# max-andr/joint-cnn-mrf

Measured on AMD Instinct MI355X. Metric: images/sec (720x480, K=9 joints) part-detector+spatial-model fwd, higher is better.
Workload: dtype f32(fp16x2 spectra, fft); 1 GPU; configs[1]: batch=64/GPU synthetic 480x720x3, part detector + spatial model forward + argmax, fp32; batch_per_gpu=64, global_batch=64, micro_batch=64, use_sm=True, collective=all_gather coords int32 [B,2,9]

## Files before the change

joint-cnn-mrf_amd/csrc/conv_fft.hip:

```cpp
#include <cmath>
#include <cstdlib>
#include <map>
#include <mutex>
#include <utility>
#include <vector>

#include "conv_fft_common.h"

namespace jcm {
namespace cfft {

template <int KS, int NP>
__global__ __launch_bounds__(256) void weight_spectra_split_kernel(const float* __restrict__ w, uint4* __restrict__ Ws, int Cin, int Cout, int CoutP, int ntl, int NY, int NX,
                                                                   int round_bf16, float* __restrict__ wscale) {
  __shared__ cf twy[192][KS - 1], twx[KS];
  const int tid = threadIdx.x;
  const int kx = blockIdx.y;
#pragma unroll 1
  for (int k = tid; k < NY * (KS - 1) + KS; k += 256) {
    const bool isy = k < NY * (KS - 1);
    const int ky = k / (KS - 1), a = isy ? k % (KS - 1) + 1 : k - NY * (KS - 1);
    const int num = isy ? (ky * a) % NY : (kx * a) % NX, den = isy ? NY : NX;
    double sn, cs;
    sincospi(-2.0 * (double)num / (double)den, &sn, &cs);
// ... 276 lines not shown
  Sizes s;
  if (!sizes_of(a.H, a.W, ks, &s)) return 0;
  return (size_t)a.B * (s.NX / 2 + 1) * a.H * a.Cout * sizeof(cf);
}
bool conv_fft_win_gather_supported(int win, int Cin) { return fft_reg_on() && cfft_rows_fwd_win_reg_supported(win, Cin); }
bool conv_fft_win_scatter_supported(int win, int Cout) { return fft_reg_on() && win == 32 && Cout % 64 == 0; }
bool conv_fft_pool_fusable(const ConvArgs& a, int ks, int ks_next) {
  Sizes s, n;
  return sizes_of(a.H, a.W, ks, &s) && sizes_of((a.H + 1) / 2, (a.W + 1) / 2, ks_next, &n) && cfft_rows_inv_pool_fwd_supported(s.NX, n.NX, a.Cout);
}
size_t conv_fft_pool_handover_bytes(const ConvArgs& a, int ks_next) {
  Sizes n;
  if (!sizes_of((a.H + 1) / 2, (a.W + 1) / 2, ks_next, &n)) return 0;
  return (size_t)a.B * (n.NX / 2 + 1) * ((a.H + 1) / 2) * a.Cout * sizeof(cf);
}
bool conv_fft_tiles_supported(const ConvArgs& a, int ks, int ks_next) {
  Sizes s;
  return fft_reg_on() && fft_tiles_on() && ks == 5 && ks_next == 5 && !a.circ && !a.win_map && a.B >= 1 && conv_fft_pool_fusable(a, ks, ks_next) &&
         a.H % 4 == 0 && a.W % 4 == 0 && sizes_of(a.H / 2, a.W / 2, ks, &s) && cfft_tiles_supported(s.NY, s.NX, a);
}
bool conv_fft_merge_fusable(const ConvArgs& a, int ks, int ks_next, const FftMerge& m, bool h16) {
  Sizes s;
  if (!conv_fft_fusable(a, ks, ks_next) || !sizes_of(a.H, a.W, ks, &s)) return false;
  const bool reg = fft_reg_on() && cfft_rows_inv_merge_fwd_reg_supported(s.NX, a, m, (ks - 1) / 2);
  return h16 ? reg : (reg || cfft_rows_inv_merge_fwd_supported(s.NX, a, m));
}
static hipError_t conv_fft_tiles_f32(const ConvArgs& a0, int ks, int np, int in_layout, void* work, const FftLink& link, hipEvent_t g0, hipEvent_t g1, hipStream_t st,
                                     const Fp16Scale* scp) {
  const void* t_in = link.t_in; void* t_next = link.t_next; const FftMerge* merge = link.merge; void* xs = link.xs; const bool xs_ready = link.xs_ready; const FftNext* nx = &link.next;
  Sizes s;
  if (np != 4 || in_layout != 0 || t_in || merge || xs || xs_ready || !t_next || !nx || !nx->pool || nx->merge || !scp || !scp->tmax || !scp->winv || !scp->tmax_next ||
      !conv_fft_tiles_supported(a0, ks, nx->ks_next) || !sizes_of(a0.H / 2, a0.W / 2, ks, &s))
    return hipErrorInvalidValue;
  ConvArgs a = a0;
  a.CoutP = pad64(a.Cout);
  const ConvArgs at = tile_view(a, s);
  const Plan3 p = plan_of(at, s, np);
  Fp16Scale sc = *scp;
  sc.hf = (float)s.NY;
  sc.nb = at.B;
  char* wk = static_cast<char*>(work);
  cf* T = reinterpret_cast<cf*>(wk);
  void* Xs = wk + align256(p.t_bytes);
  cf* Yf = reinterpret_cast<cf*>(wk + align256(p.t_bytes) + align256(p.xs_bytes));
  int dev = 0;
  if (hipError_t e = hipGetDevice(&dev); e != hipSuccess) return e;
  const cf* twb = twiddle_table(dev);
  if (!twb) return hipErrorOutOfMemory;
  if (!cfft_rows_fwd_tile_reg(s.NY, s.NX, a, T, sc.tmax, st)) return hipErrorInvalidValue;
  if (hipError_t ce = cfft_cols_fwd(s.NY, at, np, T, Xs, twb + tw_offset(s.NY), p.NXH, p.MT, sc, st); ce != hipSuccess) return ce;
  if (hipError_t e = hipGetLastError(); e != hipSuccess) return e;
  if (g0 && hipEventRecord(g0, st) != hipSuccess) return hipErrorUnknown;
  if (hipError_t e = cgemm_split(Xs, a.wp, Yf, np, p.F, at.B, a.Cin, a.Cout, p.ldy, st, 0.f); e != hipSuccess) return e;
  if (g1 && hipEventRecord(g1, st) != hipSuccess) return hipErrorUnknown;
  ConvArgs ai = at;
  ai.H = a.H / 2;
  if (!cfft_cols_inv_reg(s.NY, ai, Yf, T, p.NXH, p.ldy, (ks - 1) / 2, st, nullptr, 0.f)) return hipErrorInvalidValue;
  if (!cfft_rows_inv_pool_tile_reg(s.NY, s.NX, a, T, static_cast<cf*>(t_next), 1.0f / (float)(s.NY * s.NX), sc, st)) return hipErrorInvalidValue;
  return hipGetLastError();
}
hipError_t conv_fft_f32(const ConvArgs& a0, int ks, int np, int in_layout, int out_layout, void* work, const FftLink& link, hipEvent_t g0, hipEvent_t g1, hipStream_t st,
                        const Fp16Scale* scp) {
  if (a0.tiles) return conv_fft_tiles_f32(a0, ks, np, in_layout, work, link, g0, g1, st, scp);
  const void* t_in = link.t_in; void* t_next = link.t_next; const FftMerge* merge = link.merge; void* xs = link.xs; const bool xs_ready = link.xs_ready; const FftNext* nx = &link.next;
  Sizes s;
  if (!conv_fft_supported(a0, ks) || !sizes_of(a0.H, a0.W, ks, &s, a0.circ) || (out_layout == 2 && a0.Cout % 8) || (np != 2 && np != 4 && np != 5) || (np == 5 && a0.Cin % 32)) return hipErrorInvalidValue;
  if (a0.circ && (t_in || t_next || merge || in_layout != 0 || out_layout != 0)) return hipErrorInvalidValue;
  if (nx && (nx->pool || nx->merge) && (!t_next || (nx->pool && nx->merge))) return hipErrorInvalidValue;
  Fp16Scale sc;
  if (np >= 4) {
    if (!scp || !scp->tmax || !scp->winv || (t_next && !scp->tmax_next)) return hipErrorInvalidValue;
    sc = *scp;
    sc.hf = (float)a0.H;
    sc.nb = a0.B;
  }
  const bool h16 = sc.t16 && ((t_next && nx && nx->merge && !t_in) || (t_in && !t_next));
  if ((t_in || t_next) && !h16 && (in_layout != 0 || out_layout != 0)) return hipErrorInvalidValue;
  if (t_next && a0.Cout % CB) return hipErrorInvalidValue;
  if (sc.t16 && (np != 5 || in_layout == 0 || out_layout == 0 || xs || ((t_in || t_next) && !h16))) return hipErrorInvalidValue;
  if (merge && in_layout == 2) return hipErrorInvalidValue;
  ConvArgs a = a0;
  a.CoutP = pad64(a.Cout);
  const int opad = (ks - 1) / 2 + (a0.circ ? 4 : 0);
  const Plan3 p = plan_of(a, s, np);
  char* wk = static_cast<char*>(work);
  cf* T = reinterpret_cast<cf*>(wk);
  void* Xs = xs ? xs : wk + align256(p.t_bytes);
  cf* Yf = reinterpret_cast<cf*>(wk + align256(p.t_bytes) + align256(p.xs_bytes));
  if (sc.t16) {
    sc.t16_fwd = reinterpret_cast<float*>(wk + align256(p.t_bytes) + align256(p.xs_bytes) + align256(p.yf_bytes));
    sc.t16_inv = reinterpret_cast<float*>(wk + align256(p.t_bytes) + align256(p.xs_bytes) + align256(p.yf_bytes) + align256(p.sc_fwd_bytes));
    sc.t16_cb = p.inv_cb;
    if (t_in) sc.t16_fwd = reinterpret_cast<float*>(const_cast<char*>(static_cast<const char*>(t_in)) + align256((size_t)a.B * p.NXH * a.H * a.Cin * 4));
  }
  if (xs_ready && !xs) return hipErrorInvalidValue;
  int dev = 0;
  if (hipError_t e = hipGetDevice(&dev); e != hipSuccess) return e;
  const cf* twb = twiddle_table(dev);
  if (!twb) return hipErrorOutOfMemory;
  const cf* twx = twb + tw_offset(s.NX);
  const cf* twy = twb + tw_offset(s.NY);
  const float norm = 1.0f / (float)(s.NY * s.NX);
  const cf* Tin = t_in ? static_cast<const cf*>(t_in) : T;
  const bool fft_reg = fft_reg_on();
  if (!xs_ready) {
    if (merge && !t_in) {
      if (!(fft_reg && cfft_rows_fwd_merge_reg(s.NX, a, *merge, in_layout, T, sc.tmax, st, sc.t16_fwd))) cfft_rows_fwd_merge(s.NX, a, *merge, in_layout, T, twx, sc.tmax, st, sc.t16_fwd);
    } else if (!t_in) {
      if (a.win_map) { if (!cfft_rows_fwd_win_reg(s.NX, a, T, sc.tmax, st)) return hipErrorInvalidValue; }
      else if (!(fft_reg && cfft_rows_fwd_reg(s.NX, a, in_layout, T, sc.tmax, st, sc.t16_fwd))) cfft_rows_fwd(s.NX, a, in_layout, T, twx, sc.tmax, st, sc.t16_fwd);
    }
    if (hipError_t ce = cfft_cols_fwd(s.NY, a, np, Tin, Xs, twy, p.NXH, p.MT, sc, st); ce != hipSuccess) return ce;
  }
  if (hipError_t e = hipGetLastError(); e != hipSuccess) return e;
  if (g0 && hipEventRecord(g0, st) != hipSuccess) return hipErrorUnknown;
  const float yshift = sc.t16 ? cgemm_split_y16_shift(a.Cin) : 0.f, yinv = yshift != 0.f ? 1.0f / yshift : 0.f;
  if (hipError_t e = cgemm_split(Xs, a.wp, Yf, np, p.F, a.B, a.Cin, a.Cout, p.ldy, st, yshift); e != hipSuccess) return e;
  if (g1 && hipEventRecord(g1, st) != hipSuccess) return hipErrorUnknown;
  ConvArgs ai = a;
  if (a0.circ) { ai.H = a0.H - 8; ai.W = a0.W - 8; }
  if (!(fft_reg && p.inv_cb == 64 && cfft_cols_inv_reg(s.NY, ai, Yf, T, p.NXH, p.ldy, opad, st, sc.t16_inv, yinv))) cfft_cols_inv(s.NY, ai, Yf, T, twy, p.NXH, p.ldy, opad, st, sc.t16_inv, yinv);
  if (t_next && nx && nx->pool) {
    Sizes sn;
    if (!sizes_of((a.H + 1) / 2, (a.W + 1) / 2, nx->ks_next, &sn) ||
        !cfft_rows_inv_pool_fwd(s.NX, sn.NX, a, T, static_cast<cf*>(t_next), twx, twb + tw_offset(sn.NX), opad, norm, sc, st))
      return hipErrorInvalidValue;
  } else if (t_next && nx && nx->merge) {
    if (sc.t16) {
      float* t16n = reinterpret_cast<float*>(static_cast<char*>(t_next) + align256((size_t)a.B * p.NXH * a.H * a.Cout * 4));
      if (!(fft_reg && cfft_rows_inv_merge_fwd_reg(s.NX, a, *nx->merge, T, static_cast<cf*>(t_next), opad, norm, sc, st, t16n))) return hipErrorInvalidValue;
    } else if (!(fft_reg && cfft_rows_inv_merge_fwd_reg(s.NX, a, *nx->merge, T, static_cast<cf*>(t_next), opad, norm, sc, st)) &&
               !cfft_rows_inv_merge_fwd(s.NX, a, *nx->merge, T, static_cast<cf*>(t_next), twx, opad, norm, sc, st)) {
      return hipErrorInvalidValue;
    }
  } else if (t_next) {
    if (!(fft_reg && cfft_rows_inv_fwd_reg(s.NX, a, T, static_cast<cf*>(t_next), opad, norm, sc, st))) cfft_rows_inv_fwd(s.NX, a, T, static_cast<cf*>(t_next), twx, opad, norm, sc, st);
  } else if (!((ai.rows_mfma & 1) && cfft_rows_inv_mfma(s.NX, ai, out_layout, T, opad, norm, sc, st)) && !(fft_reg && cfft_rows_inv_reg(s.NX, ai, out_layout, T, opad, norm, sc, st))) {
    if (ai.wout_TX > 0) return hipErrorInvalidValue;
    cfft_rows_inv(s.NX, ai, out_layout, T, twx, opad, norm, sc, st);
  }
  return hipGetLastError();
}

bool conv_fft_logits_rows_supported(const ConvArgs& a, int ks) {
  Sizes s;
  return fft_logits_rows_on() && ks == 9 && !a.circ && !a.tiles && !a.win_map && conv_fft_supported(a, ks) && sizes_of(a.H, a.W, ks, &s) && cfft_logits_rows_supported(s.NX, a);
}
size_t conv_fft_logits_weight_bytes(int H, int W, int Cin) {
  Sizes s;
  return sizes_of(H, W, 9, &s) ? cfft_logits_rows_operand_bytes(s.NX, Cin) : 0;
}
size_t conv_fft_logits_workspace_bytes(const ConvArgs& a) {
  Sizes s;
  return sizes_of(a.H, a.W, 9, &s) ? align256((size_t)a.B * a.H * (s.NX / 2 + 1) * CB * sizeof(cf)) : 0;
}
hipError_t conv_fft_logits_pack(const float* w_hwio, void* aop, int H, int W, int Cin, int Cout, hipStream_t st, float* wscale) {
  Sizes s;
  if (!sizes_of(H, W, 9, &s) || Cin % 16 || Cout > 16 || !wscale) return hipErrorInvalidValue;
  if (hipError_t e = hipMemsetAsync(wscale, 0, 2 * sizeof(float), st); e != hipSuccess) return e;
  const size_t pairs = (size_t)Cin * Cout;
  const dim3 bgrid((unsigned)((pairs + 255) / 256 > 1024 ? 1024 : (pairs + 255) / 256));
  hipLaunchKernelGGL(weight_bound_kernel<81>, bgrid, dim3(256), 0, st, w_hwio, pairs, 0, wscale);
  return cfft_logits_rows_pack(s.NX, w_hwio, aop, Cin, Cout, wscale, st);
}
hipError_t conv_fft_logits_f32(const ConvArgs& a0, void* work, const FftLink& link, hipEvent_t g0, hipEvent_t g1, hipStream_t st, const Fp16Scale* scp) {
  Sizes s;
  if (!conv_fft_logits_rows_supported(a0, 9) || !sizes_of(a0.H, a0.W, 9, &s) || !link.t_in || link.t_in_16 || link.t_next || link.merge || link.xs || link.xs_ready || link.win_scatter ||
      !scp || !scp->tmax || !scp->winv || scp->common)
    return hipErrorInvalidValue;
  ConvArgs a = a0;
  a.CoutP = pad64(a.Cout);
  Fp16Scale sc = *scp;
  sc.hf = 1.f;
  sc.nb = a.B;
  int dev = 0;
  if (hipError_t e = hipGetDevice(&dev); e != hipSuccess) return e;
  const cf* twb = twiddle_table(dev);
  if (!twb) return hipErrorOutOfMemory;
  cf* S = static_cast<cf*>(work);
  if (g0 && hipEventRecord(g0, st) != hipSuccess) return hipErrorUnknown;
  if (hipError_t e = cfft_logits_rows(s.NX, a, static_cast<const cf*>(link.t_in), a.wp, sc.tmax, S, st); e != hipSuccess) return e;
  if (g1 && hipEventRecord(g1, st) != hipSuccess) return hipErrorUnknown;
  cfft_rows_inv(s.NX, a, 0, S, twb + tw_offset(s.NX), 4, 1.0f / (float)s.NX, sc, st);
  return hipGetLastError();
}

size_t conv_fft_xs_bytes(const ConvArgs& a, int ks, int np) {
  Sizes s;
  if (!sizes_of(a.H, a.W, ks, &s, a.circ)) return 0;
  return align256(plan_of(a, s, np).xs_bytes);
}
hipError_t conv_fft_spectra(const ConvArgs& a0, int ks, int np, void* work, void* xs, hipStream_t st, float* tmax, int common) {
  Sizes s;
  if (!conv_fft_supported(a0, ks) || !sizes_of(a0.H, a0.W, ks, &s, a0.circ) || !xs || (np >= 4 && !tmax)) return hipErrorInvalidValue;
  Fp16Scale sc;
  if (np >= 4) { sc.tmax = tmax; sc.hf = (float)a0.H; sc.nb = a0.B; sc.common = common; }
  ConvArgs a = a0;
  a.CoutP = pad64(a.Cout);
  const Plan3 p = plan_of(a, s, np);
  int dev = 0;
  if (hipError_t e = hipGetDevice(&dev); e != hipSuccess) return e;
  const cf* twb = twiddle_table(dev);
  if (!twb) return hipErrorOutOfMemory;
  cf* T = static_cast<cf*>(work);
  if (a.win_map) { if (!cfft_rows_fwd_win_reg(s.NX, a, T, sc.tmax, st)) return hipErrorInvalidValue; }
  else cfft_rows_fwd(s.NX, a, 0, T, twb + tw_offset(s.NX), sc.tmax, st);
  if (hipError_t ce = cfft_cols_fwd(s.NY, a, np, T, xs, twb + tw_offset(s.NY), p.NXH, p.MT, sc, st); ce != hipSuccess) return ce;
  return hipGetLastError();
}
bool conv_fft_geometry(int H, int W, int ks, int B, int Cout, int np, int* NY, int* NX, int* MT, int circ) {
  Sizes s;
  if (!sizes_of(H, W, ks, &s, circ)) return false;
  *NY = s.NY; *NX = s.NX; *MT = cgemm_split_mtile(np, B, Cout);
  return true;
}

}
```

joint-cnn-mrf_amd/csrc/conv_fft_common.h:

```cpp
#pragma once
#include "fft_lds.h"
#include "kernels.h"

namespace jcm {
namespace cfft {
using namespace fftl;
constexpr int CB = 64, NT = 256;
constexpr int kParMax = 512;

template <int N> struct Plan;
template <> struct Plan<192> { static constexpr int R1 = 8, R2 = 8, R3 = 3; };
template <> struct Plan<128> { static constexpr int R1 = 8, R2 = 4, R3 = 4; };
template <> struct Plan<100> { static constexpr int R1 = 4, R2 = 5, R3 = 5; };
template <> struct Plan<96> { static constexpr int R1 = 8, R2 = 12, R3 = 1; };
template <> struct Plan<72> { static constexpr int R1 = 8, R2 = 3, R3 = 3; };
template <> struct Plan<64> { static constexpr int R1 = 8, R2 = 8, R3 = 1; };
template <> struct Plan<60> { static constexpr int R1 = 4, R2 = 15, R3 = 1; };
template <> struct Plan<50> { static constexpr int R1 = 5, R2 = 10, R3 = 1; };
template <> struct Plan<40> { static constexpr int R1 = 8, R2 = 5, R3 = 1; };
template <> struct Plan<36> { static constexpr int R1 = 4, R2 = 3, R3 = 3; };
template <> struct Plan<32> { static constexpr int R1 = 8, R2 = 4, R3 = 1; };
template <> struct Plan<28> { static constexpr int R1 = 4, R2 = 7, R3 = 1; };
template <> struct Plan<24> { static constexpr int R1 = 8, R2 = 3, R3 = 1; };
template <> struct Plan<20> { static constexpr int R1 = 4, R2 = 5, R3 = 1; };
// ... 105 lines not shown
  float4 o[K];
  float m = 0.f;
#pragma unroll
  for (int i = 0; i < K; ++i) {
    const int t = tid + i * NTH, k = t / CH, v = t % CH;
    o[i] = make_float4(0.f, 0.f, 0.f, 0.f);
    if (t < NXH * CH) {
      const cf zk = buf[pos<NX>(k) * CH + v], zn = buf[pos<NX>(k == 0 ? 0 : NX - k) * CH + v];
      o[i] = make_float4(0.5f * (zk.x + zn.x), 0.5f * (zk.y - zn.y), 0.5f * (zk.y + zn.y), -0.5f * (zk.x - zn.x));
      m = fmaxf(fmaxf(m, fmaxf(fabsf(o[i].x), fabsf(o[i].y))), fmaxf(fabsf(o[i].z), fabsf(o[i].w)));
    }
  }
  const float s = bfp_scale(block_max_all<NTH>(m, red2, tid));
#pragma unroll
  for (int i = 0; i < K; ++i) {
    const int t = tid + i * NTH, k = t / CH, v = t % CH;
    if (t < NXH * CH) dst[t_fwd_index(k, cblk, v, b, y, B, H, C)] = make_uint2(pack_h2(o[i].x * s, o[i].y * s), pack_h2(o[i].z * s, o[i].w * s));
  }
  if (tid == 0) tinv[((size_t)b * (C / CB) + cblk) * H + y] = 1.0f / s;
  return m;
}

constexpr int kFp16TargetExp = 15;
static_assert(kFp16TargetExp <= 15, "sqrt(2) * 2^kFp16TargetExp must stay below fp16's largest number 65504");
__device__ __forceinline__ int fp16_exp(float tmax, float hf) {
  const float bound = tmax * hf;
  int e = 0;
  if (bound > 0.f && bound < 3.0e38f) (void)frexpf(bound, &e);
  return e;
}
__device__ __forceinline__ int fp16_k(float tmax, float hf) { const int k = kFp16TargetExp - fp16_exp(tmax, hf); return k > 126 ? 126 : (k < -126 ? -126 : k); }
__device__ __forceinline__ float fp16_scale(float tmax, float hf) { return ldexpf(1.f, fp16_k(tmax, hf)); }
__device__ __forceinline__ float fp16_unscale(float tmax, float hf) { return ldexpf(1.f, -fp16_k(tmax, hf)); }
__device__ __forceinline__ float tmax_of(const float* __restrict__ tmax, int b, int nb, int common) {
  if (!common) return tmax[b];
  float m = 0.f;
  for (int i = 0; i < nb; ++i) m = fmaxf(m, tmax[i]);
  return m;
}
__device__ __forceinline__ void wave_max_stash(float m, float* red) {
#pragma unroll
  for (int o = 32; o > 0; o >>= 1) m = fmaxf(m, __shfl_xor(m, o));
  if ((threadIdx.x & 63) == 0) red[threadIdx.x >> 6] = m;
}
template <int NTH>
__device__ __forceinline__ void stash_to_word(const float* red, float* dst) {
  if (threadIdx.x == 0) {
    float m = red[0];
#pragma unroll
    for (int w = 1; w < NTH / 64; ++w) m = fmaxf(m, red[w]);
    if (m > 0.f) atomicMax(reinterpret_cast<unsigned*>(dst), __float_as_uint(m));
  }
}
template <int NTH>
__device__ __forceinline__ void block_max_to(float m, float* dst, float* red, int tid) {
#pragma unroll
  for (int o = 32; o > 0; o >>= 1) m = fmaxf(m, __shfl_xor(m, o));
  if ((tid & 63) == 0) red[tid >> 6] = m;
  __syncthreads();
  if (tid == 0) {
    for (int w = 1; w < NTH / 64; ++w) m = fmaxf(m, red[w]);
    if (m > 0.f) atomicMax(reinterpret_cast<unsigned*>(dst), __float_as_uint(m));
  }
}
template <int NX> constexpr int rows_threads() { return NX >= 128 ? 512 : NX >= 72 ? 384 : 256; }
template <int NY> constexpr int colblk() { return NY > 100 ? 32 : 64; }
template <int NY> constexpr int colimg() { return NY > 96 ? 4 : 8; }
template <int NY> constexpr int colfwd_threads() { return NY * colimg<NY>() * 16 >= 8192 ? 1024 : NY * colimg<NY>() * 16 >= 4096 ? 512 : 256; }
template <int NY> constexpr int colinv_threads() { return NY * colblk<NY>() >= 4096 ? 512 : 256; }
__device__ __forceinline__ void split8h(const float (&x)[8], float scale, uint4 (&out)[2]) {
  unsigned short h[2][8];
#pragma unroll
  for (int e = 0; e < 8; ++e) {
    float v = x[e] * scale;
#pragma unroll
    for (int p = 0; p < 2; ++p) {
      const _Float16 q = static_cast<_Float16>(v);
      h[p][e] = __builtin_bit_cast(unsigned short, q);
      v = v - static_cast<float>(q);
    }
  }
#pragma unroll
  for (int p = 0; p < 2; ++p)
    out[p] = make_uint4((unsigned)h[p][0] | ((unsigned)h[p][1] << 16), (unsigned)h[p][2] | ((unsigned)h[p][3] << 16), (unsigned)h[p][4] | ((unsigned)h[p][5] << 16),
                        (unsigned)h[p][6] | ((unsigned)h[p][7] << 16));
}
__device__ __forceinline__ uint4 round8h(const float (&x)[8], float scale) {
  unsigned short h[8];
#pragma unroll
  for (int e = 0; e < 8; ++e) h[e] = __builtin_bit_cast(unsigned short, static_cast<_Float16>(x[e] * scale));
  return make_uint4((unsigned)h[0] | ((unsigned)h[1] << 16), (unsigned)h[2] | ((unsigned)h[3] << 16), (unsigned)h[4] | ((unsigned)h[5] << 16), (unsigned)h[6] | ((unsigned)h[7] << 16));
}
template <int NP>
__device__ __forceinline__ void split8(const float (&x)[8], uint4 (&out)[NP]) {
  unsigned short h[NP][8];
#pragma unroll
  for (int e = 0; e < 8; ++e) {
    float v = x[e];
#pragma unroll
    for (int p = 0; p < NP; ++p) {
      const __bf16 q = static_cast<__bf16>(v);
      h[p][e] = __builtin_bit_cast(unsigned short, q);
      v = v - static_cast<float>(q);
    }
  }
#pragma unroll
  for (int p = 0; p < NP; ++p)
    out[p] = make_uint4((unsigned)h[p][0] | ((unsigned)h[p][1] << 16), (unsigned)h[p][2] | ((unsigned)h[p][3] << 16), (unsigned)h[p][4] | ((unsigned)h[p][5] << 16),
                        (unsigned)h[p][6] | ((unsigned)h[p][7] << 16));
}
#define CFFT_BY_SIZE(N, CALL)                    \
  switch (N) {                                   \
    case 20: CALL(20); break;                    \
    case 24: CALL(24); break;                    \
    case 28: CALL(28); break;                    \
    case 32: CALL(32); break;                    \
    case 36: CALL(36); break;                    \
    case 40: CALL(40); break;                    \
    case 50: CALL(50); break;                    \
    case 60: CALL(60); break;                    \
    case 64: CALL(64); break;                    \
    case 72: CALL(72); break;                    \
    case 96: CALL(96); break;                    \
    case 100: CALL(100); break;                  \
    case 128: CALL(128); break;                  \
    default: CALL(192); break;                   \
  }

int persistent_grid(const void* kernel, int ntiles, int threads, int dyn_lds = 0);

void cfft_rows_fwd(int NX, const ConvArgs& a, int layout, cf* T, const cf* tw, float* tmax, hipStream_t st, float* t16 = nullptr);
void cfft_rows_fwd_merge(int NX, const ConvArgs& a, const FftMerge& m, int in_layout, cf* T, const cf* tw, float* tmax, hipStream_t st, float* t16 = nullptr);
hipError_t cfft_cols_fwd(int NY, const ConvArgs& a, int np, const cf* T, void* Xs, const cf* tw, int NXH, int MT, const Fp16Scale& sc, hipStream_t st);
void cfft_cols_inv(int NY, const ConvArgs& a, const cf* Yf, cf* T, const cf* tw, int NXH, int ldy, int pad, hipStream_t st, float* t16 = nullptr, float y16_inv = 0.f);
void cfft_rows_inv(int NX, const ConvArgs& a, int layout, const cf* T, const cf* tw, int pad, float norm, const Fp16Scale& sc, hipStream_t st);
bool cfft_rows_inv_reg(int NX, const ConvArgs& a, int layout, const cf* T, int pad, float norm, const Fp16Scale& sc, hipStream_t st);
bool cfft_rows_inv_fwd_reg(int NX, const ConvArgs& a, const cf* T, cf* Tn, int pad, float norm, const Fp16Scale& sc, hipStream_t st);
bool cfft_rows_fwd_reg(int NX, const ConvArgs& a, int layout, cf* T, float* tmax, hipStream_t st, float* t16);
bool cfft_rows_fwd_win_reg(int NX, const ConvArgs& a, cf* T, float* tmax, hipStream_t st);
bool cfft_rows_fwd_win_reg_supported(int NX, int Cin);
bool cfft_tiles_supported(int NY, int NX, const ConvArgs& a);
bool cfft_rows_fwd_tile_reg(int NY, int NX, const ConvArgs& a, cf* T, float* tmax, hipStream_t st);
bool cfft_rows_inv_pool_tile_reg(int NY, int NX, const ConvArgs& a, const cf* T, cf* Tn, float norm, const Fp16Scale& sc, hipStream_t st);
bool cfft_rows_fwd_merge_reg(int NX, const ConvArgs& a, const FftMerge& m, int in_layout, cf* T, float* tmax, hipStream_t st, float* t16);
bool cfft_cols_inv_reg(int NY, const ConvArgs& a, const cf* Yf, cf* T, int NXH, int ldy, int pad, hipStream_t st, float* t16, float y16_inv = 0.f);
void cfft_rows_inv_fwd(int NX, const ConvArgs& a, const cf* T, cf* Tn, const cf* tw, int pad, float norm, const Fp16Scale& sc, hipStream_t st);
bool cfft_rows_inv_pool_fwd(int NXI, int NXO, const ConvArgs& a, const cf* T, cf* Tn, const cf* twi, const cf* two, int pad, float norm, const Fp16Scale& sc, hipStream_t st);
bool cfft_rows_inv_merge_fwd(int NX, const ConvArgs& a, const FftMerge& m, const cf* T, cf* Tn, const cf* tw, int pad, float norm, const Fp16Scale& sc, hipStream_t st);
bool cfft_rows_inv_merge_fwd_reg(int NX, const ConvArgs& a, const FftMerge& m, const cf* T, cf* Tn, int pad, float norm, const Fp16Scale& sc, hipStream_t st, float* t16n = nullptr);
bool cfft_rows_inv_merge_fwd_reg_supported(int NX, const ConvArgs& a, const FftMerge& m, int pad);
bool cfft_rows_inv_pool_fwd_supported(int NXI, int NXO, int Cout);
bool cfft_rows_inv_mfma(int NX, const ConvArgs& a, int layout, const cf* T, int pad, float norm, const Fp16Scale& sc, hipStream_t st);
bool cfft_rows_inv_merge_fwd_supported(int NX, const ConvArgs& a, const FftMerge& m);
bool cfft_logits_rows_supported(int NX, const ConvArgs& a);
size_t cfft_logits_rows_operand_bytes(int NX, int Cin);
hipError_t cfft_logits_rows_pack(int NX, const float* w_hwio, void* aop, int Cin, int Cout, float* wscale, hipStream_t st);
hipError_t cfft_logits_rows(int NX, const ConvArgs& a, const cf* T, const void* aop, const float* tmax, cf* S, hipStream_t st);
}
}
```

joint-cnn-mrf_amd/csrc/conv_fft_logits.hip:

```cpp
#include "conv_fft_common.h"

namespace jcm {
namespace cfft {

constexpr int kLrWaves = 8, kLrRows = 72, kLrUnits = 8;
constexpr int kLrLds = kLrWaves * kLrRows * kLrUnits * 16;
typedef _Float16 f16x8 __attribute__((ext_vector_type(8)));
typedef float f32x4 __attribute__((ext_vector_type(4)));

__device__ __forceinline__ int lr_slot(int r, int u) { return r * kLrUnits + (u ^ ((r >> 1) & 7)); }

__global__ __launch_bounds__(256) void logits_rows_operand_kernel(const float* __restrict__ w, uint4* __restrict__ Aop, int Cin, int Cout, int NX, float* __restrict__ wscale) {
  __shared__ cf twx[9];
  const int kx = blockIdx.y, KC = Cin >> 4;
  if (threadIdx.x < 9) {
    double sn, cs;
    sincospi(-2.0 * (double)((kx * (int)threadIdx.x) % NX) / (double)NX, &sn, &cs);
    twx[threadIdx.x] = cf{(float)cs, (float)sn};
  }
  __syncthreads();
  int ex = 0;
  const float bound = wscale[0];
  if (bound > 0.f && bound < 3.0e38f) (void)frexpf(bound, &ex);
  const float wmul = ldexpf(1.f, 14 - ex);
  if (blockIdx.x == 0 && blockIdx.y == 0 && threadIdx.x == 0) wscale[1] = ldexpf(1.f, ex - 14);
  const int e = blockIdx.x * 256 + threadIdx.x;
  if (e >= 9 * KC * 64) return;
  const int lane = e & 63, c = (e >> 6) % KC, dy = (e >> 6) / KC;
  const int j = lane & 15, g = lane >> 4, ch0 = c * 16 + (g & 1) * 8;
  cf a[8];
#pragma unroll
  for (int i = 0; i < 8; ++i) a[i] = cf{0.f, 0.f};
  if (j < Cout) {
#pragma unroll
    for (int b = 0; b < 9; ++b) {
      const float* tap = w + ((size_t)(dy * 9 + (8 - b)) * Cin + ch0) * Cout + j;
      const cf tw = twx[b];
#pragma unroll
      for (int i = 0; i < 8; ++i) a[i] = sfma(tap[(size_t)i * Cout], tw, a[i]);
    }
  }
  float vr[8], vi[8];
#pragma unroll
  for (int i = 0; i < 8; ++i) {
    vr[i] = g < 2 ? a[i].x : -a[i].y;
    vi[i] = g < 2 ? a[i].y : a[i].x;
  }
  uint4 u[2];
  uint4* dst = Aop + ((((size_t)kx * 9 + dy) * KC + c) * 4) * 64 + lane;
  split8h(vr, wmul, u);
  dst[0] = u[0]; dst[64] = u[1];
  split8h(vi, wmul, u);
  dst[128] = u[0]; dst[192] = u[1];
}

__global__ __launch_bounds__(512) __attribute__((amdgpu_waves_per_eu(4, 4))) void logits_rows_kernel(const float4* __restrict__ T, const uint4* __restrict__ Aop,
                                                                                                       const float* __restrict__ tmax, cf* __restrict__ S, int B, int H, int KC,
                                                                                                       int NXH, int per) {
  extern __shared__ __attribute__((aligned(16))) char lr_smem[];
  const int xcd = blockIdx.x & 7, slot = blockIdx.x >> 3, item = xcd * per + slot;
  if (slot >= per || item >= NXH * B) return;
  const int kx = item / B, b = item - kx * B;
  const int tid = threadIdx.x, wave = tid >> 6, lane = tid & 63;
  uint4* wl = reinterpret_cast<uint4*>(lr_smem) + wave * (kLrRows * kLrUnits);
  for (int i = lane; i < kLrRows * kLrUnits; i += 64) wl[i] = make_uint4(0u, 0u, 0u, 0u);
  const float scale = fp16_scale(tmax[b], 1.f);
  f32x4 sr[4], si[4];
#pragma unroll
  for (int m = 0; m < 4; ++m) { sr[m] = f32x4{0.f, 0.f, 0.f, 0.f}; si[m] = f32x4{0.f, 0.f, 0.f, 0.f}; }
  const int y0 = lane >> 1, y1 = 32 + (lane >> 1), hh = lane & 1;
  const bool in0 = y0 < H, in1 = y1 < H;
  float4 pre[2][4];
  auto fetch = [&](int c) __attribute__((always_inline)) {
    const float4* src = T + (((size_t)kx * KC + c) * B + b) * H * 8 + hh * 4;
#pragma unroll
    for (int q = 0; q < 4; ++q) {
      pre[0][q] = in0 ? src[(size_t)y0 * 8 + q] : make_float4(0.f, 0.f, 0.f, 0.f);
      pre[1][q] = in1 ? src[(size_t)y1 * 8 + q] : make_float4(0.f, 0.f, 0.f, 0.f);
    }
  };
  auto stash = [&](int i, int y) __attribute__((always_inline)) {
    float re[8], im[8];
#pragma unroll
    for (int q = 0; q < 4; ++q) { re[2 * q] = pre[i][q].x; im[2 * q] = pre[i][q].y; re[2 * q + 1] = pre[i][q].z; im[2 * q + 1] = pre[i][q].w; }
    uint4 ur[2], ui[2];
    split8h(re, scale, ur);
    split8h(im, scale, ui);
    const int r = y + 4;
    wl[lr_slot(r, hh)] = ur[0]; wl[lr_slot(r, 2 + hh)] = ui[0];
    wl[lr_slot(r, 4 + hh)] = ur[1]; wl[lr_slot(r, 6 + hh)] = ui[1];
  };
  const int g = lane >> 4, rl = lane & 15;
  if (wave < KC) fetch(wave);
  for (int c = wave; c < KC; c += kLrWaves) {
    if (in0) stash(0, y0);
    if (in1) stash(1, y1);
    if (c + kLrWaves < KC) fetch(c + kLrWaves);
    __builtin_amdgcn_fence(__ATOMIC_RELEASE, "wavefront");
    __builtin_amdgcn_wave_barrier();
    __builtin_amdgcn_fence(__ATOMIC_ACQUIRE, "wavefront");
    const uint4* bp = Aop + (((size_t)kx * 9 * KC + c) * 4) * 64 + lane;
#pragma unroll 3
    for (int dy = 0; dy < 9; ++dy) {
      const uint4* bq = bp + (size_t)dy * KC * 256;
      const f16x8 br0 = __builtin_bit_cast(f16x8, bq[0]), br1 = __builtin_bit_cast(f16x8, bq[64]);
      const f16x8 bi0 = __builtin_bit_cast(f16x8, bq[128]), bi1 = __builtin_bit_cast(f16x8, bq[192]);
#pragma unroll
      for (int m = 0; m < 4; ++m) {
        const int r = m * 16 + rl + dy;
        const f16x8 a0 = __builtin_bit_cast(f16x8, wl[lr_slot(r, g)]), a1 = __builtin_bit_cast(f16x8, wl[lr_slot(r, 4 + g)]);
        sr[m] = __builtin_amdgcn_mfma_f32_16x16x32_f16(a0, br1, sr[m], 0, 0, 0);
        si[m] = __builtin_amdgcn_mfma_f32_16x16x32_f16(a0, bi1, si[m], 0, 0, 0);
        sr[m] = __builtin_amdgcn_mfma_f32_16x16x32_f16(a1, br0, sr[m], 0, 0, 0);
        si[m] = __builtin_amdgcn_mfma_f32_16x16x32_f16(a1, bi0, si[m], 0, 0, 0);
        sr[m] = __builtin_amdgcn_mfma_f32_16x16x32_f16(a0, br0, sr[m], 0, 0, 0);
        si[m] = __builtin_amdgcn_mfma_f32_16x16x32_f16(a0, bi0, si[m], 0, 0, 0);
      }
    }
    __builtin_amdgcn_fence(__ATOMIC_RELEASE, "wavefront");
    __builtin_amdgcn_wave_barrier();
    __builtin_amdgcn_fence(__ATOMIC_ACQUIRE, "wavefront");
  }
  __syncthreads();
  float* red = reinterpret_cast<float*>(lr_smem);
#pragma unroll
  for (int m = 0; m < 4; ++m)
#pragma unroll
    for (int i = 0; i < 4; ++i) {
      red[(wave * 32 + m * 4 + i) * 64 + lane] = sr[m][i];
      red[(wave * 32 + 16 + m * 4 + i) * 64 + lane] = si[m][i];
    }
  __syncthreads();
  cf* Sb = S + ((size_t)b * H * NXH + kx) * 64;
#pragma unroll
  for (int q = 0; q < 2; ++q) {
    const int pi = tid + 512 * q, lo = pi & 63, mi = pi >> 6;
    float re = 0.f, im = 0.f;
#pragma unroll
    for (int wv = 0; wv < kLrWaves; ++wv) {
      re += red[(wv * 32 + mi) * 64 + lo];
      im += red[(wv * 32 + 16 + mi) * 64 + lo];
    }
    const int row = (mi >> 2) * 16 + (lo >> 4) * 4 + (mi & 3);
    if (row < H) Sb[(size_t)row * NXH * 64 + (lo & 15)] = cf{re, im};
  }
  for (int e = tid; e < H * 24; e += 512) {
    const int row = e / 24, q = e - row * 24;
    *reinterpret_cast<float4*>(Sb + (size_t)row * NXH * 64 + 16 + 2 * q) = make_float4(0.f, 0.f, 0.f, 0.f);
  }
}

bool cfft_logits_rows_supported(int NX, const ConvArgs& a) { return NX == 96 && a.H >= 1 && a.H <= 64 && a.Cin % 16 == 0 && a.Cout >= 1 && a.Cout <= 16 && a.B >= 1; }
size_t cfft_logits_rows_operand_bytes(int NX, int Cin) { return (size_t)(NX / 2 + 1) * 9 * (Cin / 16) * 4 * 64 * sizeof(uint4); }
hipError_t cfft_logits_rows_pack(int NX, const float* w_hwio, void* aop, int Cin, int Cout, float* wscale, hipStream_t st) {
  const dim3 grid((unsigned)((9 * (Cin / 16) * 64 + 255) / 256), (unsigned)(NX / 2 + 1));
  hipLaunchKernelGGL(logits_rows_operand_kernel, grid, dim3(256), 0, st, w_hwio, static_cast<uint4*>(aop), Cin, Cout, NX, wscale);
  return hipGetLastError();
}
hipError_t cfft_logits_rows(int NX, const ConvArgs& a, const cf* T, const void* aop, const float* tmax, cf* S, hipStream_t st) {
  if (!cfft_logits_rows_supported(NX, a)) return hipErrorInvalidValue;
  static LdsAttr attr;
  if (hipError_t e = attr.ensure(reinterpret_cast<const void*>(logits_rows_kernel), kLrLds); e != hipSuccess) return e;
  const int NXH = NX / 2 + 1, items = NXH * a.B, per = (items + 7) / 8;
  hipLaunchKernelGGL(logits_rows_kernel, dim3((unsigned)(per * 8)), dim3(512), kLrLds, st, reinterpret_cast<const float4*>(T), static_cast<const uint4*>(aop), tmax, S, a.B, a.H,
                     a.Cin / 16, NXH, per);
  return hipGetLastError();
}

}
}
```

Before: 7317 images/sec.

## Batch two images per logits-rows block, narrow spectra to 16 columns, add dedicated inverse

The logits channel-GEMM kernel now processes G=2 batch images per work group. Each weight operand fetched from global memory is reused across two images' MFMA chains, with grouped prefetch and sched barriers, at the cost of halved occupancy and doubled LDS. The spectrum buffer is narrowed from 64 to 16 complex columns per row, which removes the zero-padding stores. A new specialised inverse-row FFT kernel packs 4 rows per block into the transform's channel lanes to match the narrow layout. An environment variable can switch back to G=1.

```diff
diff --git a/joint-cnn-mrf_amd/csrc/conv_fft.hip b/joint-cnn-mrf_amd/csrc/conv_fft.hip
--- a/joint-cnn-mrf_amd/csrc/conv_fft.hip
+++ b/joint-cnn-mrf_amd/csrc/conv_fft.hip
@@ -452,7 +452,7 @@
 }
 size_t conv_fft_logits_workspace_bytes(const ConvArgs& a) {
   Sizes s;
-  return sizes_of(a.H, a.W, 9, &s) ? align256((size_t)a.B * a.H * (s.NX / 2 + 1) * CB * sizeof(cf)) : 0;
+  return sizes_of(a.H, a.W, 9, &s) ? align256((size_t)a.B * a.H * (s.NX / 2 + 1) * kLrCols * sizeof(cf)) : 0;
 }
 hipError_t conv_fft_logits_pack(const float* w_hwio, void* aop, int H, int W, int Cin, int Cout, hipStream_t st, float* wscale) {
   Sizes s;
@@ -468,8 +468,7 @@
   if (!conv_fft_logits_rows_supported(a0, 9) || !sizes_of(a0.H, a0.W, 9, &s) || !link.t_in || link.t_in_16 || link.t_next || link.merge || link.xs || link.xs_ready || link.win_scatter ||
       !scp || !scp->tmax || !scp->winv || scp->common)
     return hipErrorInvalidValue;
-  ConvArgs a = a0;
-  a.CoutP = pad64(a.Cout);
+  const ConvArgs& a = a0;
   Fp16Scale sc = *scp;
   sc.hf = 1.f;
   sc.nb = a.B;
@@ -481,8 +480,7 @@
   if (g0 && hipEventRecord(g0, st) != hipSuccess) return hipErrorUnknown;
   if (hipError_t e = cfft_logits_rows(s.NX, a, static_cast<const cf*>(link.t_in), a.wp, sc.tmax, S, st); e != hipSuccess) return e;
   if (g1 && hipEventRecord(g1, st) != hipSuccess) return hipErrorUnknown;
-  cfft_rows_inv(s.NX, a, 0, S, twb + tw_offset(s.NX), 4, 1.0f / (float)s.NX, sc, st);
-  return hipGetLastError();
+  return cfft_logits_rows_inv(s.NX, a, S, twb + tw_offset(s.NX), 4, 1.0f / (float)s.NX, sc, st);
 }
 
 size_t conv_fft_xs_bytes(const ConvArgs& a, int ks, int np) {
diff --git a/joint-cnn-mrf_amd/csrc/conv_fft_common.h b/joint-cnn-mrf_amd/csrc/conv_fft_common.h
--- a/joint-cnn-mrf_amd/csrc/conv_fft_common.h
+++ b/joint-cnn-mrf_amd/csrc/conv_fft_common.h
@@ -281,9 +281,11 @@
 bool cfft_rows_inv_pool_fwd_supported(int NXI, int NXO, int Cout);
 bool cfft_rows_inv_mfma(int NX, const ConvArgs& a, int layout, const cf* T, int pad, float norm, const Fp16Scale& sc, hipStream_t st);
 bool cfft_rows_inv_merge_fwd_supported(int NX, const ConvArgs& a, const FftMerge& m);
+constexpr int kLrCols = 16;
 bool cfft_logits_rows_supported(int NX, const ConvArgs& a);
 size_t cfft_logits_rows_operand_bytes(int NX, int Cin);
 hipError_t cfft_logits_rows_pack(int NX, const float* w_hwio, void* aop, int Cin, int Cout, float* wscale, hipStream_t st);
 hipError_t cfft_logits_rows(int NX, const ConvArgs& a, const cf* T, const void* aop, const float* tmax, cf* S, hipStream_t st);
-}
-}
+hipError_t cfft_logits_rows_inv(int NX, const ConvArgs& a, const cf* S, const cf* tw, int pad, float norm, const Fp16Scale& sc, hipStream_t st);
+}
+}
diff --git a/joint-cnn-mrf_amd/csrc/conv_fft_logits.hip b/joint-cnn-mrf_amd/csrc/conv_fft_logits.hip
--- a/joint-cnn-mrf_amd/csrc/conv_fft_logits.hip
+++ b/joint-cnn-mrf_amd/csrc/conv_fft_logits.hip
@@ -1,10 +1,15 @@
+#include <cstdlib>
+#include <type_traits>
+
 #include "conv_fft_common.h"
 
 namespace jcm {
 namespace cfft {
 
 constexpr int kLrWaves = 8, kLrRows = 72, kLrUnits = 8;
-constexpr int kLrLds = kLrWaves * kLrRows * kLrUnits * 16;
+constexpr int kLrSlice = kLrRows * kLrUnits;
+constexpr int kLrLds = kLrWaves * kLrSlice * 16;
+constexpr int kLrGroup = 2;
 typedef _Float16 f16x8 __attribute__((ext_vector_type(8)));
 typedef float f32x4 __attribute__((ext_vector_type(4)));
 
@@ -54,68 +59,108 @@
   dst[128] = u[0]; dst[192] = u[1];
 }
 
-__global__ __launch_bounds__(512) __attribute__((amdgpu_waves_per_eu(4, 4))) void logits_rows_kernel(const float4* __restrict__ T, const uint4* __restrict__ Aop,
-                                                                                                       const float* __restrict__ tmax, cf* __restrict__ S, int B, int H, int KC,
-                                                                                                       int NXH, int per) {
+template <int G>
+__global__ __launch_bounds__(512) __attribute__((amdgpu_waves_per_eu(4 / G, 4 / G))) void logits_rows_kernel(const float4* __restrict__ T, const uint4* __restrict__ Aop,
+                                                                                                               const float* __restrict__ tmax, cf* __restrict__ S, int B, int H,
+                                                                                                               int KC, int NXH, int per) {
   extern __shared__ __attribute__((aligned(16))) char lr_smem[];
+  const int NG = (B + G - 1) / G;
   const int xcd = blockIdx.x & 7, slot = blockIdx.x >> 3, item = xcd * per + slot;
-  if (slot >= per || item >= NXH * B) return;
-  const int kx = item / B, b = item - kx * B;
+  if (slot >= per || item >= NXH * NG) return;
+  const int kx = item / NG, b0 = (item - kx * NG) * G, ng = B - b0 < G ? B - b0 : G;
   const int tid = threadIdx.x, wave = tid >> 6, lane = tid & 63;
-  uint4* wl = reinterpret_cast<uint4*>(lr_smem) + wave * (kLrRows * kLrUnits);
-  for (int i = lane; i < kLrRows * kLrUnits; i += 64) wl[i] = make_uint4(0u, 0u, 0u, 0u);
-  const float scale = fp16_scale(tmax[b], 1.f);
-  f32x4 sr[4], si[4];
-#pragma unroll
-  for (int m = 0; m < 4; ++m) { sr[m] = f32x4{0.f, 0.f, 0.f, 0.f}; si[m] = f32x4{0.f, 0.f, 0.f, 0.f}; }
+  uint4* wl = reinterpret_cast<uint4*>(lr_smem) + wave * (G * kLrSlice);
+  for (int i = lane; i < G * kLrSlice; i += 64) wl[i] = make_uint4(0u, 0u, 0u, 0u);
+  float scale[G];
+  f32x4 sr[G][4], si[G][4];
+#pragma unroll
+  for (int gi = 0; gi < G; ++gi) {
+    scale[gi] = gi < ng ? fp16_scale(tmax[b0 + gi], 1.f) : 1.f;
+#pragma unroll
+    for (int m = 0; m < 4; ++m) { sr[gi][m] = f32x4{0.f, 0.f, 0.f, 0.f}; si[gi][m] = f32x4{0.f, 0.f, 0.f, 0.f}; }
+  }
   const int y0 = lane >> 1, y1 = 32 + (lane >> 1), hh = lane & 1;
   const bool in0 = y0 < H, in1 = y1 < H;
-  float4 pre[2][4];
+  float4 pre[G][2][4];
+  const int yl0 = in0 ? y0 : H - 1, yl1 = in1 ? y1 : H - 1;
   auto fetch = [&](int c) __attribute__((always_inline)) {
-    const float4* src = T + (((size_t)kx * KC + c) * B + b) * H * 8 + hh * 4;
-#pragma unroll
-    for (int q = 0; q < 4; ++q) {
-      pre[0][q] = in0 ? src[(size_t)y0 * 8 + q] : make_float4(0.f, 0.f, 0.f, 0.f);
-      pre[1][q] = in1 ? src[(size_t)y1 * 8 + q] : make_float4(0.f, 0.f, 0.f, 0.f);
+#pragma unroll
+    for (int gi = 0; gi < G; ++gi) {
+      const float4* src = T + (((size_t)kx * KC + c) * B + (gi < ng ? b0 + gi : B - 1)) * H * 8 + hh * 4;
+#pragma unroll
+      for (int q = 0; q < 4; ++q) {
+        pre[gi][0][q] = src[(size_t)yl0 * 8 + q];
+        pre[gi][1][q] = src[(size_t)yl1 * 8 + q];
+      }
     }
   };
-  auto stash = [&](int i, int y) __attribute__((always_inline)) {
+  auto stash = [&](int gi, int i, int y) __attribute__((always_inline)) {
     float re[8], im[8];
 #pragma unroll
-    for (int q = 0; q < 4; ++q) { re[2 * q] = pre[i][q].x; im[2 * q] = pre[i][q].y; re[2 * q + 1] = pre[i][q].z; im[2 * q + 1] = pre[i][q].w; }
+    for (int q = 0; q < 4; ++q) { re[2 * q] = pre[gi][i][q].x; im[2 * q] = pre[gi][i][q].y; re[2 * q + 1] = pre[gi][i][q].z; im[2 * q + 1] = pre[gi][i][q].w; }
     uint4 ur[2], ui[2];
-    split8h(re, scale, ur);
-    split8h(im, scale, ui);
+    split8h(re, scale[gi], ur);
+    split8h(im, scale[gi], ui);
     const int r = y + 4;
-    wl[lr_slot(r, hh)] = ur[0]; wl[lr_slot(r, 2 + hh)] = ui[0];
-    wl[lr_slot(r, 4 + hh)] = ur[1]; wl[lr_slot(r, 6 + hh)] = ui[1];
+    uint4* wg = wl + gi * kLrSlice;
+    wg[lr_slot(r, hh)] = ur[0]; wg[lr_slot(r, 2 + hh)] = ui[0];
+    wg[lr_slot(r, 4 + hh)] = ur[1]; wg[lr_slot(r, 6 + hh)] = ui[1];
   };
   const int g = lane >> 4, rl = lane & 15;
   if (wave < KC) fetch(wave);
   for (int c = wave; c < KC; c += kLrWaves) {
-    if (in0) stash(0, y0);
-    if (in1) stash(1, y1);
-    if (c + kLrWaves < KC) fetch(c + kLrWaves);
+#pragma unroll
+    for (int gi = 0; gi < G; ++gi) {
+      if (gi < ng) {
+        if (in0) stash(gi, 0, y0);
+        if (in1) stash(gi, 1, y1);
+      }
+    }
     __builtin_amdgcn_fence(__ATOMIC_RELEASE, "wavefront");
     __builtin_amdgcn_wave_barrier();
     __builtin_amdgcn_fence(__ATOMIC_ACQUIRE, "wavefront");
     const uint4* bp = Aop + (((size_t)kx * 9 * KC + c) * 4) * 64 + lane;
+    const bool more = c + kLrWaves < KC;
+    auto group = [&](int d3, auto dg, bool pf) __attribute__((always_inline)) {
+      constexpr int DG = decltype(dg)::value;
+      if constexpr (DG > 1) __builtin_amdgcn_sched_barrier(0);
+      uint4 bf[DG][4];
+#pragma unroll
+      for (int d = 0; d < DG; ++d)
+#pragma unroll
+        for (int f = 0; f < 4; ++f) bf[d][f] = bp[(size_t)(d3 + d) * KC * 256 + f * 64];
+      if (pf) fetch(c + kLrWaves);
+      if constexpr (DG > 1) __builtin_amdgcn_sched_barrier(0);
+#pragma unroll
+      for (int d = 0; d < DG; ++d) {
+        const int dy = d3 + d;
+        const f16x8 br0 = __builtin_bit_cast(f16x8, bf[d][0]), br1 = __builtin_bit_cast(f16x8, bf[d][1]);
+        const f16x8 bi0 = __builtin_bit_cast(f16x8, bf[d][2]), bi1 = __builtin_bit_cast(f16x8, bf[d][3]);
+#pragma unroll
+        for (int m = 0; m < 4; ++m) {
+          const int r = m * 16 + rl + dy;
+#pragma unroll
+          for (int gi = 0; gi < G; ++gi) {
+            const uint4* wg = wl + gi * kLrSlice;
+            const f16x8 a0 = __builtin_bit_cast(f16x8, wg[lr_slot(r, g)]), a1 = __builtin_bit_cast(f16x8, wg[lr_slot(r, 4 + g)]);
+            sr[gi][m] = __builtin_amdgcn_mfma_f32_16x16x32_f16(a0, br1, sr[gi][m], 0, 0, 0);
+            si[gi][m] = __builtin_amdgcn_mfma_f32_16x16x32_f16(a0, bi1, si[gi][m], 0, 0, 0);
+            sr[gi][m] = __builtin_amdgcn_mfma_f32_16x16x32_f16(a1, br0, sr[gi][m], 0, 0, 0);
+            si[gi][m] = __builtin_amdgcn_mfma_f32_16x16x32_f16(a1, bi0, si[gi][m], 0, 0, 0);
+            sr[gi][m] = __builtin_amdgcn_mfma_f32_16x16x32_f16(a0, br0, sr[gi][m], 0, 0, 0);
+            si[gi][m] = __builtin_amdgcn_mfma_f32_16x16x32_f16(a0, bi0, si[gi][m], 0, 0, 0);
+          }
+        }
+      }
+    };
+    using std::integral_constant;
+    if constexpr (G == 1) {
+      if (more) fetch(c + kLrWaves);
 #pragma unroll 3
-    for (int dy = 0; dy < 9; ++dy) {
-      const uint4* bq = bp + (size_t)dy * KC * 256;
-      const f16x8 br0 = __builtin_bit_cast(f16x8, bq[0]), br1 = __builtin_bit_cast(f16x8, bq[64]);
-      const f16x8 bi0 = __builtin_bit_cast(f16x8, bq[128]), bi1 = __builtin_bit_cast(f16x8, bq[192]);
-#pragma unroll
-      for (int m = 0; m < 4; ++m) {
-        const int r = m * 16 + rl + dy;
-        const f16x8 a0 = __builtin_bit_cast(f16x8, wl[lr_slot(r, g)]), a1 = __builtin_bit_cast(f16x8, wl[lr_slot(r, 4 + g)]);
-        sr[m] = __builtin_amdgcn_mfma_f32_16x16x32_f16(a0, br1, sr[m], 0, 0, 0);
-        si[m] = __builtin_amdgcn_mfma_f32_16x16x32_f16(a0, bi1, si[m], 0, 0, 0);
-        sr[m] = __builtin_amdgcn_mfma_f32_16x16x32_f16(a1, br0, sr[m], 0, 0, 0);
-        si[m] = __builtin_amdgcn_mfma_f32_16x16x32_f16(a1, bi0, si[m], 0, 0, 0);
-        sr[m] = __builtin_amdgcn_mfma_f32_16x16x32_f16(a0, br0, sr[m], 0, 0, 0);
-        si[m] = __builtin_amdgcn_mfma_f32_16x16x32_f16(a0, bi0, si[m], 0, 0, 0);
-      }
+      for (int dy = 0; dy < 9; ++dy) group(dy, integral_constant<int, 1>{}, false);
+    } else {
+#pragma unroll 1
+      for (int d3 = 0; d3 < 9; d3 += 3) group(d3, integral_constant<int, 3>{}, d3 == 6 && more);
     }
     __builtin_amdgcn_fence(__ATOMIC_RELEASE, "wavefront");
     __builtin_amdgcn_wave_barrier();
@@ -124,30 +169,81 @@
   __syncthreads();
   float* red = reinterpret_cast<float*>(lr_smem);
 #pragma unroll
-  for (int m = 0; m < 4; ++m)
-#pragma unroll
-    for (int i = 0; i < 4; ++i) {
-      red[(wave * 32 + m * 4 + i) * 64 + lane] = sr[m][i];
-      red[(wave * 32 + 16 + m * 4 + i) * 64 + lane] = si[m][i];
-    }
-  __syncthreads();
-  cf* Sb = S + ((size_t)b * H * NXH + kx) * 64;
-#pragma unroll
-  for (int q = 0; q < 2; ++q) {
-    const int pi = tid + 512 * q, lo = pi & 63, mi = pi >> 6;
-    float re = 0.f, im = 0.f;
-#pragma unroll
-    for (int wv = 0; wv < kLrWaves; ++wv) {
-      re += red[(wv * 32 + mi) * 64 + lo];
-      im += red[(wv * 32 + 16 + mi) * 64 + lo];
-    }
-    const int row = (mi >> 2) * 16 + (lo >> 4) * 4 + (mi & 3);
-    if (row < H) Sb[(size_t)row * NXH * 64 + (lo & 15)] = cf{re, im};
-  }
-  for (int e = tid; e < H * 24; e += 512) {
-    const int row = e / 24, q = e - row * 24;
-    *reinterpret_cast<float4*>(Sb + (size_t)row * NXH * 64 + 16 + 2 * q) = make_float4(0.f, 0.f, 0.f, 0.f);
-  }
+  for (int gi = 0; gi < G; ++gi)
+#pragma unroll
+    for (int m = 0; m < 4; ++m)
+#pragma unroll
+      for (int i = 0; i < 4; ++i) {
+        red[((gi * kLrWaves + wave) * 32 + m * 4 + i) * 64 + lane] = sr[gi][m][i];
+        red[((gi * kLrWaves + wave) * 32 + 16 + m * 4 + i) * 64 + lane] = si[gi][m][i];
+      }
+  __syncthreads();
+#pragma unroll
+  for (int gi = 0; gi < G; ++gi) {
+    if (gi >= ng) break;
+    cf* Sb = S + ((size_t)(b0 + gi) * H * NXH + kx) * kLrCols;
+    const float* rg = red + gi * (kLrWaves * 32 * 64);
+#pragma unroll
+    for (int q = 0; q < 2; ++q) {
+      const int pi = tid + 512 * q, lo = pi & 63, mi = pi >> 6;
+      float re = 0.f, im = 0.f;
+#pragma unroll
+      for (int wv = 0; wv < kLrWaves; ++wv) {
+        re += rg[(wv * 32 + mi) * 64 + lo];
+        im += rg[(wv * 32 + 16 + mi) * 64 + lo];
+      }
+      const int row = (mi >> 2) * 16 + (lo >> 4) * 4 + (mi & 3);
+      if (row < H) Sb[(size_t)row * NXH * kLrCols + (lo & 15)] = cf{re, im};
+    }
+  }
+}
+
+constexpr int kLiRows = 4;
+__global__ __launch_bounds__(rows_threads<96>()) void logits_rows_inv_kernel(const cf* __restrict__ S, float* __restrict__ out, const cf* __restrict__ twg, const float* __restrict__ bias,
+                                                                             const float* __restrict__ scale, const float* __restrict__ shift, int relu_bn, int BH, int H, int W, int Cout,
+                                                                             int pad, float norm0, Fp16Scale sc) {
+  constexpr int NX = 96, CH = CB / 2, NXH = NX / 2 + 1, NTR = rows_threads<NX>(), K = (NXH * CH + NTR - 1) / NTR, CP = kLrCols / 2;
+  static_assert(CH == kLiRows * CP, "the rows of a work group fill the transform's channel lanes");
+  __shared__ cf buf[NX * CH];
+  __shared__ cf tw[NX];
+  const int tid = threadIdx.x, by0 = blockIdx.x * kLiRows;
+  twiddles<NX, NTR>(tw, twg, tid);
+  const float4* src = reinterpret_cast<const float4*>(S);
+#pragma unroll
+  for (int i = 0; i < K; ++i) {
+    const int t = tid + i * NTR, k = t / CH, v = t % CH, by = by0 + v / CP;
+    if (t < NXH * CH) {
+      float4 q = by < BH ? src[((size_t)by * NXH + k) * CP + v % CP] : make_float4(0.f, 0.f, 0.f, 0.f);
+      const bool edge = k == 0 || k == NX / 2;
+      if (edge) { q.y = 0.f; q.w = 0.f; }
+      buf[k * CH + v] = cf{q.x - q.w, q.y + q.z};
+      if (!edge) buf[(NX - k) * CH + v] = cf{q.x + q.w, q.z - q.y};
+    }
+  }
+  __syncthreads();
+  fft<NX, 1, CH, NTR>(buf, tw, tid);
+  const int v = tid % CH, by = by0 + v / CP, c = 2 * (v % CP);
+  if (by < BH && c < Cout) {
+    const float ncommon = norm0 * sc.winv[0];
+    const float norm = ncommon * fp16_unscale(sc.tmax[by / H], sc.hf);
+    const bool two = c + 1 < Cout, pairs = (Cout & 1) == 0;
+    const float b0v = bias[c], b1v = two ? bias[c + 1] : 0.f;
+    float s0 = 1.f, s1 = 1.f, h0 = 0.f, h1 = 0.f;
+    if (relu_bn) { s0 = scale[c]; h0 = shift[c]; if (two) { s1 = scale[c + 1]; h1 = shift[c + 1]; } }
+    for (int x = tid / CH; x < W; x += NTR / CH) {
+      const cf z = buf[pos<NX>(x + pad) * CH + v];
+      float v0 = z.x * norm + b0v, v1 = z.y * norm + b1v;
+      if (relu_bn) { v0 = fmaxf(v0, 0.f) * s0 + h0; v1 = fmaxf(v1, 0.f) * s1 + h1; }
+      float* o = out + ((size_t)by * W + x) * Cout + c;
+      if (pairs) *reinterpret_cast<cf*>(o) = cf{v0, v1};
+      else { o[0] = v0; if (two) o[1] = v1; }
+    }
+  }
+}
+
+static int logits_group() {
+  static const int g = [] { const char* e = std::getenv("JCM_FFT_LOGITS_GROUP"); return e && std::atoi(e) == 1 ? 1 : kLrGroup; }();
+  return g;
 }
 
 bool cfft_logits_rows_supported(int NX, const ConvArgs& a) { return NX == 96 && a.H >= 1 && a.H <= 64 && a.Cin % 16 == 0 && a.Cout >= 1 && a.Cout <= 16 && a.B >= 1; }
@@ -157,13 +253,23 @@
   hipLaunchKernelGGL(logits_rows_operand_kernel, grid, dim3(256), 0, st, w_hwio, static_cast<uint4*>(aop), Cin, Cout, NX, wscale);
   return hipGetLastError();
 }
+template <int G> static hipError_t launch_logits_rows(const ConvArgs& a, int NXH, const cf* T, const void* aop, const float* tmax, cf* S, hipStream_t st) {
+  static LdsAttr attr;
+  if (hipError_t e = attr.ensure(reinterpret_cast<const void*>(logits_rows_kernel<G>), G * kLrLds); e != hipSuccess) return e;
+  const int items = NXH * ((a.B + G - 1) / G), per = (items + 7) / 8;
+  hipLaunchKernelGGL(logits_rows_kernel<G>, dim3((unsigned)(per * 8)), dim3(512), G * kLrLds, st, reinterpret_cast<const float4*>(T), static_cast<const uint4*>(aop), tmax, S, a.B, a.H,
+                     a.Cin / 16, NXH, per);
+  return hipGetLastError();
+}
 hipError_t cfft_logits_rows(int NX, const ConvArgs& a, const cf* T, const void* aop, const float* tmax, cf* S, hipStream_t st) {
   if (!cfft_logits_rows_supported(NX, a)) return hipErrorInvalidValue;
-  static LdsAttr attr;
-  if (hipError_t e = attr.ensure(reinterpret_cast<const void*>(logits_rows_kernel), kLrLds); e != hipSuccess) return e;
-  const int NXH = NX / 2 + 1, items = NXH * a.B, per = (items + 7) / 8;
-  hipLaunchKernelGGL(logits_rows_kernel, dim3((unsigned)(per * 8)), dim3(512), kLrLds, st, reinterpret_cast<const float4*>(T), static_cast<const uint4*>(aop), tmax, S, a.B, a.H,
-                     a.Cin / 16, NXH, per);
+  return logits_group() == 1 ? launch_logits_rows<1>(a, NX / 2 + 1, T, aop, tmax, S, st) : launch_logits_rows<kLrGroup>(a, NX / 2 + 1, T, aop, tmax, S, st);
+}
+hipError_t cfft_logits_rows_inv(int NX, const ConvArgs& a, const cf* S, const cf* tw, int pad, float norm, const Fp16Scale& sc, hipStream_t st) {
+  if (!cfft_logits_rows_supported(NX, a) || !sc.tmax || !sc.winv || sc.common) return hipErrorInvalidValue;
+  const int BH = a.B * a.H;
+  hipLaunchKernelGGL(logits_rows_inv_kernel, dim3((unsigned)((BH + kLiRows - 1) / kLiRows)), dim3(rows_threads<96>()), 0, st, S, static_cast<float*>(a.out), tw, a.bias, a.scale, a.shift,
+                     a.relu_bn, BH, a.H, a.W, a.Cout, pad, norm, sc);
   return hipGetLastError();
 }
 
```

Result: no change. 7347 images/sec (median of 5 runs) (+0.4%).
